# jspenmar/slowtv_monodepth

Hardware: AMD Instinct MI355X
Metric: training images/sec (640×192, 3-frame) at 1/2/4/8 MI355X; warp+SSIM HBM GB/s (higher is better)
Workload: dtype f32

## Files before the change

slowtv_monodepth_amd/csrc/smd_conv_stem.hip:

```cpp
#include "smd_common.h"
#include "smd_kernels.h"
#include "smd_conv_mfma_dev.h"
#include <algorithm>

namespace smd {

namespace {

template <int C> struct StemFwd {
  static constexpr int NI = 7*C, NS = (NI + 1)/2;
  static constexpr int PR = 13, PD = 67, PITCH = 68;
  static constexpr int PLANE = C*PR*PITCH, ITEMS = C*PR*PD;
};

template <int C>
__global__ __launch_bounds__(256) void k_stem_pack_w(const float* __restrict__ w, uint4* __restrict__ wp) {
  using T = StemFwd<C>;
  const int idx = blockIdx.x*256 + threadIdx.x;
  if (idx >= 2*T::NS*64) return;
  const int lane = idx & 63, s = (idx >> 6) % T::NS, mt = idx/(64*T::NS);
  const int i = 2*s + (lane >> 5), co = mt*32 + (lane & 31);
  float v[8];
#pragma unroll
  for (int kx = 0; kx < 8; ++kx) v[kx] = (i < T::NI && kx < 7) ? w[((size_t)co*T::NI + i)*7 + kx] : 0.f;
  unsigned pk[4][3];
#pragma unroll
  for (int q = 0; q < 4; ++q) split_pair<3>(v[2*q], v[2*q + 1], pk[q]);
#pragma unroll
  for (int p = 0; p < 3; ++p) wp[((size_t)(mt*T::NS + s)*3 + p)*64 + lane] = uint4{pk[0][p], pk[1][p], pk[2][p], pk[3][p]};
}

template <int C>
__global__ __launch_bounds__(256, 2) void k_stem_fwd(const float* __restrict__ x, const uint4* __restrict__ wp, float* __restrict__ y, int H, int W, int ho, int wo) {
  using T = StemFwd<C>;
  constexpr int NS = T::NS, NI = T::NI, PR = T::PR, PD = T::PD, PITCH = T::PITCH, PLANE = T::PLANE, ITEMS = T::ITEMS;
  __shared__ __attribute__((aligned(16))) unsigned xs[3*PLANE];
  const int lane = threadIdx.x & 63, wv = __builtin_amdgcn_readfirstlane(threadIdx.x >> 6), j = lane & 31, g = lane >> 5;
  const int x0 = blockIdx.x*64, y0 = blockIdx.y*4, b = blockIdx.z;
  const float* xb = x + (size_t)b*C*H*W;

  for (int base = 0; base < ITEMS; base += 1024) {
    float v[4][2];
#pragma unroll
    for (int u = 0; u < 4; ++u) {
      const int item = base + u*256 + (int)threadIdx.x;
      const int d = item % PD, r = (item/PD) % PR, c = item/(PD*PR);
      const int gy = 2*y0 - 3 + r, gx = 2*x0 - 3 + 2*d;
      const bool ok = item < ITEMS && gy >= 0 && gy < H;
      v[u][0] = (ok && gx >= 0 && gx < W) ? xb[((size_t)c*H + gy)*W + gx] : 0.f;
      v[u][1] = (ok && gx + 1 >= 0 && gx + 1 < W) ? xb[((size_t)c*H + gy)*W + gx + 1] : 0.f;
    }
#pragma unroll
    for (int u = 0; u < 4; ++u) {
      const int item = base + u*256 + (int)threadIdx.x;
      if (item < ITEMS) {
        const int d = item % PD, rc = item/PD;
        unsigned pk[3];
        split_pair<3>(v[u][0], v[u][1], pk);
#pragma unroll
        for (int p = 0; p < 3; ++p) xs[p*PLANE + rc*PITCH + d] = pk[p];
      }
    }
  }
  __syncthreads();

  f32x16 acc[2][2], lo[2][2];
#pragma unroll
  for (int mt = 0; mt < 2; ++mt)
#pragma unroll
    for (int nf = 0; nf < 2; ++nf)
#pragma unroll
      for (int r = 0; r < 16; ++r) { acc[mt][nf][r] = 0.f; lo[mt][nf][r] = 0.f; }

  const uint4* wl = wp + lane;
  uint4 an[2][3];
#pragma unroll
  for (int mt = 0; mt < 2; ++mt)
#pragma unroll
    for (int p = 0; p < 3; ++p) an[mt][p] = wl[((mt*NS + 0)*3 + p)*64];
#pragma unroll
  for (int s = 0; s < NS; ++s) {
    bf16x8 A[2][3];
#pragma unroll
    for (int mt = 0; mt < 2; ++mt)
#pragma unroll
      for (int p = 0; p < 3; ++p) A[mt][p] = as_frag(an[mt][p]);
    const int sn = min(s + 1, NS - 1);
#pragma unroll
    for (int mt = 0; mt < 2; ++mt)
#pragma unroll
      for (int p = 0; p < 3; ++p) an[mt][p] = wl[((mt*NS + sn)*3 + p)*64];
    const int i = min(2*s + g, NI - 1);
    const int c = i/7, ky = i - 7*c;
    const unsigned* row = xs + (c*PR + 2*wv + ky)*PITCH + j;
    bf16x8 Bf[2][3];
#pragma unroll
    for (int nf = 0; nf < 2; ++nf)
#pragma unroll
      for (int p = 0; p < 3; ++p) {
        const unsigned* q = row + p*PLANE + nf*32;
        Bf[nf][p] = as_frag(uint4{q[0], q[1], q[2], q[3]});
      }
    split_mfma<3>(A, Bf, acc, lo);
  }

  const int yy = y0 + wv;
  if (yy >= ho) return;
#pragma unroll
  for (int mt = 0; mt < 2; ++mt)
#pragma unroll
    for (int nf = 0; nf < 2; ++nf) {
      const int xx = x0 + nf*32 + j;
      if (xx < wo) {
#pragma unroll
        for (int r = 0; r < 16; ++r) {
          const int co = mt*32 + mfma32_row(r, g);
          y[(((size_t)b*64 + co)*ho + yy)*wo + xx] = acc[mt][nf][r] + lo[mt][nf][r];
        }
      }
    }
}

template <int C> struct StemWgrad {
  static constexpr int NW = 49*C, NT = (NW + 31)/32, NTW = (NT + 1)/2;
  static constexpr int XP = 34, GP = 36;
  static constexpr int XPLANE = C*8*2*XP, GPLANE = 64*GP;
  static constexpr int XITEMS = C*2*XP, XTR = (XITEMS + 255)/256;
};

template <int C>
__global__ __launch_bounds__(256, 2) void k_stem_wgrad(const float* __restrict__ x, const float* __restrict__ gy, float* __restrict__ partial,
                                                       int H, int W, int ho, int wo, int rows_per_block) {
  using T = StemWgrad<C>;
  constexpr int NW = T::NW, NT = T::NT, NTW = T::NTW, XP = T::XP, GP = T::GP, XPLANE = T::XPLANE, GPLANE = T::GPLANE, XITEMS = T::XITEMS, XTR = T::XTR;
  constexpr int NPROD = n_products(3);
  __shared__ __attribute__((aligned(16))) unsigned xs[3*XPLANE];
  __shared__ __attribute__((aligned(16))) unsigned gs[3*GPLANE];
  const int lane = threadIdx.x & 63, wv = __builtin_amdgcn_readfirstlane(threadIdx.x >> 6), j = lane & 31, g = lane >> 5;
  const int mt = wv & 1, nh = wv >> 1;
  const int x0 = blockIdx.x*64, ybeg = blockIdx.y*rows_per_block, nrows = min(rows_per_block, ho - ybeg), b = blockIdx.z;
  const float* xb = x + (size_t)b*C*H*W;
  const float* gb = gy + (size_t)b*64*ho*wo;

  int xoff[NTW], sh[NTW], kyv[NTW];
#pragma unroll
  for (int i = 0; i < NTW; ++i) {
    const int n = min((nh + 2*i)*32 + j, NW - 1);
    const int c = n/49, rem = n - 49*c, ky = rem/7, kx = rem - 7*ky;
    xoff[i] = (c*16 + ((kx & 1) ^ 1))*XP; sh[i] = (kx + 1) >> 1; kyv[i] = ky;
  }

  float xv[XTR][4], gv[4][4];
  auto load_x = [&](int ir0) {
#pragma unroll
    for (int t = 0; t < XTR; ++t) {
      const int item = t*256 + (int)threadIdx.x;
      const int d = item % XP, rr = (item/XP) & 1, c = item/(2*XP);
      const int ir = ir0 + rr, gc = 2*x0 - 4 + 4*d;
      const bool ok = item < XITEMS && ir >= 0 && ir < H;
#pragma unroll
      for (int k = 0; k < 4; ++k) xv[t][k] = (ok && gc + k >= 0 && gc + k < W) ? xb[((size_t)c*H + ir)*W + gc + k] : 0.f;
    }
  };
  auto file_x = [&](int ir0) {
#pragma unroll
    for (int t = 0; t < XTR; ++t) {
      const int item = t*256 + (int)threadIdx.x;
      if (item < XITEMS) {
        const int d = item % XP, rr = (item/XP) & 1, c = item/(2*XP);
        const int slot = (ir0 + rr + 8) & 7;
        unsigned pe[3], po[3];
        split_pair<3>(xv[t][0], xv[t][2], pe);
        split_pair<3>(xv[t][1], xv[t][3], po);
#pragma unroll
        for (int p = 0; p < 3; ++p) {
          xs[p*XPLANE + ((c*8 + slot)*2 + 0)*XP + d] = pe[p];
          xs[p*XPLANE + ((c*8 + slot)*2 + 1)*XP + d] = po[p];
        }
      }
    }
  };
  auto load_g = [&](int yy) {
#pragma unroll
    for (int t = 0; t < 4; ++t) {
      const int item = t*256 + (int)threadIdx.x;
      const int co = item >> 4, xa = x0 + 4*(item & 15);
#pragma unroll
      for (int k = 0; k < 4; ++k) gv[t][k] = (xa + k < wo) ? gb[((size_t)co*ho + yy)*wo + xa + k] : 0.f;
    }
  };
  auto file_g = [&]() {
#pragma unroll
    for (int t = 0; t < 4; ++t) {
      const int item = t*256 + (int)threadIdx.x;
      const int co = item >> 4, q = item & 15;
      unsigned p0[3], p1[3];
      split_pair<3>(gv[t][0], gv[t][1], p0);
      split_pair<3>(gv[t][2], gv[t][3], p1);
#pragma unroll
      for (int p = 0; p < 3; ++p) {
        gs[p*GPLANE + co*GP + 2*q] = p0[p];
        gs[p*GPLANE + co*GP + 2*q + 1] = p1[p];
      }
    }
  };

  f32x16 acc[NTW];
#pragma unroll
  for (int i = 0; i < NTW; ++i)
#pragma unroll
    for (int r = 0; r < 16; ++r) acc[i][r] = 0.f;

  for (int k = 0; k < 4; ++k) { load_x(2*ybeg - 4 + 2*k); file_x(2*ybeg - 4 + 2*k); }
  load_g(ybeg); file_g();
  __syncthreads();
  for (int r = 0; r < nrows; ++r) {
    const int yy = ybeg + r;
    const bool more = r + 1 < nrows;
    if (more) { load_x(2*yy + 4); load_g(yy + 1); }
    unsigned rowa[NTW];
#pragma unroll
    for (int i = 0; i < NTW; ++i) rowa[i] = (unsigned)(xoff[i] + ((2*yy + 5 + kyv[i]) & 7)*2*XP);
#pragma unroll
    for (int ks = 0; ks < 4; ++ks) {
      bf16x8 A[3];
#pragma unroll
      for (int p = 0; p < 3; ++p) A[p] = as_frag(*reinterpret_cast<const uint4*>(&gs[p*GPLANE + (mt*32 + j)*GP + ks*8 + g*4]));
#pragma unroll
      for (int i = 0; i < NTW; ++i) {
        if (nh + 2*i >= NT) continue;
        const int e = ks*16 + g*8 + sh[i];
        const unsigned* q = xs + rowa[i] + (e >> 1);
        const unsigned s16 = (unsigned)(e & 1)*16u;
        bf16x8 Bf[3];
#pragma unroll
        for (int p = 0; p < 3; ++p) {
          const unsigned d0 = q[p*XPLANE], d1 = q[p*XPLANE + 1], d2 = q[p*XPLANE + 2], d3 = q[p*XPLANE + 3], d4 = q[p*XPLANE + 4];
          Bf[p] = as_frag(uint4{__builtin_amdgcn_alignbit(d1, d0, s16), __builtin_amdgcn_alignbit(d2, d1, s16),
                                __builtin_amdgcn_alignbit(d3, d2, s16), __builtin_amdgcn_alignbit(d4, d3, s16)});
        }
#pragma unroll
        for (int t = 0; t < NPROD; ++t) acc[i] = mfma_bf16(A[prod_a(3, t)], Bf[prod_b(3, t)], acc[i]);
      }
    }
    __syncthreads();
    if (more) { file_x(2*yy + 4); file_g(); }
    __syncthreads();
  }

  const size_t blk = ((size_t)b*gridDim.y + blockIdx.y)*gridDim.x + blockIdx.x;
#pragma unroll
  for (int i = 0; i < NTW; ++i) {
    const int nt = nh + 2*i, n = nt*32 + j;
    if (nt < NT && n < NW) {
#pragma unroll
      for (int r = 0; r < 16; ++r) {
        const int co = mt*32 + mfma32_row(r, g);
        partial[(blk*64 + co)*NW + n] = acc[i][r];
      }
    }
  }
}

void stem_wgrad_shape(int B, int ho, int wo, dim3& grid, int& rows) {
  const int strips = ceil_div(wo, 64);
  const long long units = (long long)strips*B;
  const int groups = (int)std::max(1ll, std::min<long long>(ceil_div(ho, 8), 512/std::max(units, 1ll)));
  rows = ceil_div(ho, groups);
  grid = dim3(strips, ceil_div(ho, rows), B);
}

}

bool conv_stem_served(int C, int CO) { return CO == 64 && (C == 3 || C == 6); }
size_t conv_stem_packed_bytes(int C) { return (size_t)2*((7*C + 1)/2)*3*1024; }
size_t conv_stem_wgrad_floats(int B, int C, int H, int W) {
  dim3 grid; int rows;
  stem_wgrad_shape(B, (H - 1)/2 + 1, (W - 1)/2 + 1, grid, rows);
  return partial_sets_floats(grid.x*grid.y*grid.z, (size_t)64*49*C);
}
hipError_t launch_conv_stem_pack(const float* w, void* wp, int C, hipStream_t st) {
  const int n = 2*((7*C + 1)/2)*64;
  if (C == 3) hipLaunchKernelGGL(k_stem_pack_w<3>, dim3(ceil_div(n, 256)), dim3(256), 0, st, w, (uint4*)wp);
  else hipLaunchKernelGGL(k_stem_pack_w<6>, dim3(ceil_div(n, 256)), dim3(256), 0, st, w, (uint4*)wp);
  return hipGetLastError();
}
hipError_t launch_conv_stem_fwd(const float* x, const void* wp, float* y, int B, int C, int H, int W, hipStream_t st) {
  const int ho = (H - 1)/2 + 1, wo = (W - 1)/2 + 1;
  const dim3 grid(ceil_div(wo, 64), ceil_div(ho, 4), B);
  if (C == 3) hipLaunchKernelGGL(k_stem_fwd<3>, grid, dim3(256), 0, st, x, (const uint4*)wp, y, H, W, ho, wo);
  else hipLaunchKernelGGL(k_stem_fwd<6>, grid, dim3(256), 0, st, x, (const uint4*)wp, y, H, W, ho, wo);
  return hipGetLastError();
}
hipError_t launch_conv_stem_bwd_wgt(const float* x, const float* gy, float* g_w, float* partial, int B, int C, int H, int W, hipStream_t st) {
  const int ho = (H - 1)/2 + 1, wo = (W - 1)/2 + 1, n = 64*49*C;
  dim3 grid; int rows;
  stem_wgrad_shape(B, ho, wo, grid, rows);
  if (C == 3) hipLaunchKernelGGL(k_stem_wgrad<3>, grid, dim3(256), 0, st, x, gy, partial, H, W, ho, wo, rows);
  else hipLaunchKernelGGL(k_stem_wgrad<6>, grid, dim3(256), 0, st, x, gy, partial, H, W, ho, wo, rows);
  return launch_partial_sets_finalize(partial, grid.x*grid.y*grid.z, n, SetIndexMap{}, g_w, st);
}

}
```

Baseline: 953.8.

## Restructure stem conv kernels: triple-buffered weight prefetch, split odd tile, compact row ring

In the stem forward kernel, the input tile staging loop is fully unrolled. Weight fragments are now prefetched two steps ahead through a three-slot register ring, with scheduling barriers around the MFMA step. In the weight-gradient kernel, the x row ring shrinks from 8 slots to 5 row pairs, and global loads are made unconditional through clamped addresses, with masking moved to the LDS fill. The A fragments for all k-steps are hoisted before the MFMA loop. When the tile count is odd, the last tile's k-steps are split across the two wave halves and combined through LDS. These changes aim to balance MFMA work across waves and overlap global loads with compute, at the cost of more registers and extra barriers.

Result: no change. 955.9, median of 3 (+0.2%).

```diff
diff --git a/slowtv_monodepth_amd/csrc/smd_conv_stem.hip b/slowtv_monodepth_amd/csrc/smd_conv_stem.hip
--- a/slowtv_monodepth_amd/csrc/smd_conv_stem.hip
+++ b/slowtv_monodepth_amd/csrc/smd_conv_stem.hip
@@ -10,7 +10,7 @@
 template <int C> struct StemFwd {
   static constexpr int NI = 7*C, NS = (NI + 1)/2;
   static constexpr int PR = 13, PD = 67, PITCH = 68;
-  static constexpr int PLANE = C*PR*PITCH, ITEMS = C*PR*PD;
+  static constexpr int PLANE = C*PR*PITCH, ITEMS = C*PR*PD, TRIPS = (ITEMS + 255)/256;
 };
 
 template <int C>
@@ -33,30 +33,30 @@
 template <int C>
 __global__ __launch_bounds__(256, 2) void k_stem_fwd(const float* __restrict__ x, const uint4* __restrict__ wp, float* __restrict__ y, int H, int W, int ho, int wo) {
   using T = StemFwd<C>;
-  constexpr int NS = T::NS, NI = T::NI, PR = T::PR, PD = T::PD, PITCH = T::PITCH, PLANE = T::PLANE, ITEMS = T::ITEMS;
+  constexpr int NS = T::NS, NI = T::NI, PR = T::PR, PD = T::PD, PITCH = T::PITCH, PLANE = T::PLANE, ITEMS = T::ITEMS, TRIPS = T::TRIPS;
   __shared__ __attribute__((aligned(16))) unsigned xs[3*PLANE];
   const int lane = threadIdx.x & 63, wv = __builtin_amdgcn_readfirstlane(threadIdx.x >> 6), j = lane & 31, g = lane >> 5;
   const int x0 = blockIdx.x*64, y0 = blockIdx.y*4, b = blockIdx.z;
   const float* xb = x + (size_t)b*C*H*W;
 
-  for (int base = 0; base < ITEMS; base += 1024) {
-    float v[4][2];
-#pragma unroll
-    for (int u = 0; u < 4; ++u) {
-      const int item = base + u*256 + (int)threadIdx.x;
+  {
+    float v[TRIPS][2];
+#pragma unroll
+    for (int t = 0; t < TRIPS; ++t) {
+      const int item = t*256 + (int)threadIdx.x;
       const int d = item % PD, r = (item/PD) % PR, c = item/(PD*PR);
       const int gy = 2*y0 - 3 + r, gx = 2*x0 - 3 + 2*d;
       const bool ok = item < ITEMS && gy >= 0 && gy < H;
-      v[u][0] = (ok && gx >= 0 && gx < W) ? xb[((size_t)c*H + gy)*W + gx] : 0.f;
-      v[u][1] = (ok && gx + 1 >= 0 && gx + 1 < W) ? xb[((size_t)c*H + gy)*W + gx + 1] : 0.f;
-    }
-#pragma unroll
-    for (int u = 0; u < 4; ++u) {
-      const int item = base + u*256 + (int)threadIdx.x;
+      v[t][0] = (ok && gx >= 0 && gx < W) ? xb[((size_t)c*H + gy)*W + gx] : 0.f;
+      v[t][1] = (ok && gx + 1 >= 0 && gx + 1 < W) ? xb[((size_t)c*H + gy)*W + gx + 1] : 0.f;
+    }
+#pragma unroll
+    for (int t = 0; t < TRIPS; ++t) {
+      const int item = t*256 + (int)threadIdx.x;
       if (item < ITEMS) {
         const int d = item % PD, rc = item/PD;
         unsigned pk[3];
-        split_pair<3>(v[u][0], v[u][1], pk);
+        split_pair<3>(v[t][0], v[t][1], pk);
 #pragma unroll
         for (int p = 0; p < 3; ++p) xs[p*PLANE + rc*PITCH + d] = pk[p];
       }
@@ -73,23 +73,17 @@
       for (int r = 0; r < 16; ++r) { acc[mt][nf][r] = 0.f; lo[mt][nf][r] = 0.f; }
 
   const uint4* wl = wp + lane;
-  uint4 an[2][3];
-#pragma unroll
-  for (int mt = 0; mt < 2; ++mt)
-#pragma unroll
-    for (int p = 0; p < 3; ++p) an[mt][p] = wl[((mt*NS + 0)*3 + p)*64];
+  bf16x8 A[3][2][3];
+  auto fetch_a = [&](bf16x8 (&dst)[2][3], int s) {
+#pragma unroll
+    for (int mt = 0; mt < 2; ++mt)
+#pragma unroll
+      for (int p = 0; p < 3; ++p) dst[mt][p] = as_frag(wl[((mt*NS + s)*3 + p)*64]);
+  };
+  fetch_a(A[0], 0); fetch_a(A[1], 1);
 #pragma unroll
   for (int s = 0; s < NS; ++s) {
-    bf16x8 A[2][3];
-#pragma unroll
-    for (int mt = 0; mt < 2; ++mt)
-#pragma unroll
-      for (int p = 0; p < 3; ++p) A[mt][p] = as_frag(an[mt][p]);
-    const int sn = min(s + 1, NS - 1);
-#pragma unroll
-    for (int mt = 0; mt < 2; ++mt)
-#pragma unroll
-      for (int p = 0; p < 3; ++p) an[mt][p] = wl[((mt*NS + sn)*3 + p)*64];
+    if (s + 2 < NS) fetch_a(A[(s + 2) % 3], s + 2);
     const int i = min(2*s + g, NI - 1);
     const int c = i/7, ky = i - 7*c;
     const unsigned* row = xs + (c*PR + 2*wv + ky)*PITCH + j;
@@ -101,7 +95,8 @@
         const unsigned* q = row + p*PLANE + nf*32;
         Bf[nf][p] = as_frag(uint4{q[0], q[1], q[2], q[3]});
       }
-    split_mfma<3>(A, Bf, acc, lo);
+    split_mfma<3>(A[s % 3], Bf, acc, lo);
+    __builtin_amdgcn_sched_barrier(0);
   }
 
   const int yy = y0 + wv;
@@ -123,8 +118,10 @@
 
 template <int C> struct StemWgrad {
   static constexpr int NW = 49*C, NT = (NW + 31)/32, NTW = (NT + 1)/2;
+  static constexpr bool SPLIT = NT & 1;
   static constexpr int XP = 34, GP = 36;
-  static constexpr int XPLANE = C*8*2*XP, GPLANE = 64*GP;
+  static constexpr int RP = 5;
+  static constexpr int XPLANE = C*RP*2*2*XP, GPLANE = 64*GP;
   static constexpr int XITEMS = C*2*XP, XTR = (XITEMS + 255)/256;
 };
 
@@ -132,7 +129,8 @@
 __global__ __launch_bounds__(256, 2) void k_stem_wgrad(const float* __restrict__ x, const float* __restrict__ gy, float* __restrict__ partial,
                                                        int H, int W, int ho, int wo, int rows_per_block) {
   using T = StemWgrad<C>;
-  constexpr int NW = T::NW, NT = T::NT, NTW = T::NTW, XP = T::XP, GP = T::GP, XPLANE = T::XPLANE, GPLANE = T::GPLANE, XITEMS = T::XITEMS, XTR = T::XTR;
+  constexpr int NW = T::NW, NT = T::NT, NTW = T::NTW, XP = T::XP, GP = T::GP, XPLANE = T::XPLANE, GPLANE = T::GPLANE, XITEMS = T::XITEMS, XTR = T::XTR, RP = T::RP;
+  constexpr bool SPLIT = T::SPLIT;
   constexpr int NPROD = n_products(3);
   __shared__ __attribute__((aligned(16))) unsigned xs[3*XPLANE];
   __shared__ __attribute__((aligned(16))) unsigned gs[3*GPLANE];
@@ -142,12 +140,13 @@
   const float* xb = x + (size_t)b*C*H*W;
   const float* gb = gy + (size_t)b*64*ho*wo;
 
-  int xoff[NTW], sh[NTW], kyv[NTW];
+  auto tile_of = [&](int i) { return (SPLIT && i == NTW - 1) ? NT - 1 : nh + 2*i; };
+  int xoff[NTW], sh[NTW], dpair[NTW];
 #pragma unroll
   for (int i = 0; i < NTW; ++i) {
-    const int n = min((nh + 2*i)*32 + j, NW - 1);
+    const int n = min(tile_of(i)*32 + j, NW - 1);
     const int c = n/49, rem = n - 49*c, ky = rem/7, kx = rem - 7*ky;
-    xoff[i] = (c*16 + ((kx & 1) ^ 1))*XP; sh[i] = (kx + 1) >> 1; kyv[i] = ky;
+    xoff[i] = ((c*RP*2 + ((ky + 1) & 1))*2 + ((kx & 1) ^ 1))*XP; sh[i] = (kx + 1) >> 1; dpair[i] = RP + ((ky - 3) >> 1);
   }
 
   float xv[XTR][4], gv[4][4];
@@ -157,25 +156,29 @@
       const int item = t*256 + (int)threadIdx.x;
       const int d = item % XP, rr = (item/XP) & 1, c = item/(2*XP);
       const int ir = ir0 + rr, gc = 2*x0 - 4 + 4*d;
-      const bool ok = item < XITEMS && ir >= 0 && ir < H;
-#pragma unroll
-      for (int k = 0; k < 4; ++k) xv[t][k] = (ok && gc + k >= 0 && gc + k < W) ? xb[((size_t)c*H + ir)*W + gc + k] : 0.f;
-    }
-  };
-  auto file_x = [&](int ir0) {
+      const float* row = xb + ((size_t)min(c, C - 1)*H + min(max(ir, 0), H - 1))*W;
+#pragma unroll
+      for (int k = 0; k < 4; ++k) xv[t][k] = row[min(max(gc + k, 0), W - 1)];
+    }
+  };
+  auto file_x = [&](int ir0, int slot) {
 #pragma unroll
     for (int t = 0; t < XTR; ++t) {
       const int item = t*256 + (int)threadIdx.x;
       if (item < XITEMS) {
         const int d = item % XP, rr = (item/XP) & 1, c = item/(2*XP);
-        const int slot = (ir0 + rr + 8) & 7;
+        const int ir = ir0 + rr, gc = 2*x0 - 4 + 4*d;
+        const bool ok = ir >= 0 && ir < H;
+        float z[4];
+#pragma unroll
+        for (int k = 0; k < 4; ++k) z[k] = (ok && gc + k >= 0 && gc + k < W) ? xv[t][k] : 0.f;
         unsigned pe[3], po[3];
-        split_pair<3>(xv[t][0], xv[t][2], pe);
-        split_pair<3>(xv[t][1], xv[t][3], po);
+        split_pair<3>(z[0], z[2], pe);
+        split_pair<3>(z[1], z[3], po);
 #pragma unroll
         for (int p = 0; p < 3; ++p) {
-          xs[p*XPLANE + ((c*8 + slot)*2 + 0)*XP + d] = pe[p];
-          xs[p*XPLANE + ((c*8 + slot)*2 + 1)*XP + d] = po[p];
+          xs[p*XPLANE + (((c*RP + slot)*2 + rr)*2 + 0)*XP + d] = pe[p];
+          xs[p*XPLANE + (((c*RP + slot)*2 + rr)*2 + 1)*XP + d] = po[p];
         }
       }
     }
@@ -186,17 +189,20 @@
       const int item = t*256 + (int)threadIdx.x;
       const int co = item >> 4, xa = x0 + 4*(item & 15);
 #pragma unroll
-      for (int k = 0; k < 4; ++k) gv[t][k] = (xa + k < wo) ? gb[((size_t)co*ho + yy)*wo + xa + k] : 0.f;
+      for (int k = 0; k < 4; ++k) gv[t][k] = gb[((size_t)co*ho + yy)*wo + min(xa + k, wo - 1)];
     }
   };
   auto file_g = [&]() {
 #pragma unroll
     for (int t = 0; t < 4; ++t) {
       const int item = t*256 + (int)threadIdx.x;
-      const int co = item >> 4, q = item & 15;
+      const int co = item >> 4, q = item & 15, xa = x0 + 4*q;
+      float z[4];
+#pragma unroll
+      for (int k = 0; k < 4; ++k) z[k] = (xa + k < wo) ? gv[t][k] : 0.f;
       unsigned p0[3], p1[3];
-      split_pair<3>(gv[t][0], gv[t][1], p0);
-      split_pair<3>(gv[t][2], gv[t][3], p1);
+      split_pair<3>(z[0], z[1], p0);
+      split_pair<3>(z[2], z[3], p1);
 #pragma unroll
       for (int p = 0; p < 3; ++p) {
         gs[p*GPLANE + co*GP + 2*q] = p0[p];
@@ -211,24 +217,33 @@
 #pragma unroll
     for (int r = 0; r < 16; ++r) acc[i][r] = 0.f;
 
-  for (int k = 0; k < 4; ++k) { load_x(2*ybeg - 4 + 2*k); file_x(2*ybeg - 4 + 2*k); }
+  int ym = ybeg % RP;
+  for (int k = 0; k < 4; ++k) { load_x(2*ybeg - 4 + 2*k); file_x(2*ybeg - 4 + 2*k, (ym + RP - 2 + k) % RP); }
   load_g(ybeg); file_g();
   __syncthreads();
   for (int r = 0; r < nrows; ++r) {
     const int yy = ybeg + r;
     const bool more = r + 1 < nrows;
+    bf16x8 A[4][3];
+#pragma unroll
+    for (int ks = 0; ks < 4; ++ks)
+#pragma unroll
+      for (int p = 0; p < 3; ++p) A[ks][p] = as_frag(*reinterpret_cast<const uint4*>(&gs[p*GPLANE + (mt*32 + j)*GP + ks*8 + g*4]));
     if (more) { load_x(2*yy + 4); load_g(yy + 1); }
+    __syncthreads();
+    __builtin_amdgcn_sched_barrier(0);
     unsigned rowa[NTW];
 #pragma unroll
-    for (int i = 0; i < NTW; ++i) rowa[i] = (unsigned)(xoff[i] + ((2*yy + 5 + kyv[i]) & 7)*2*XP);
+    for (int i = 0; i < NTW; ++i) {
+      int slot = ym + dpair[i];
+      slot -= slot >= RP ? RP : 0; slot -= slot >= RP ? RP : 0;
+      rowa[i] = (unsigned)(xoff[i] + slot*4*XP);
+    }
 #pragma unroll
     for (int ks = 0; ks < 4; ++ks) {
-      bf16x8 A[3];
-#pragma unroll
-      for (int p = 0; p < 3; ++p) A[p] = as_frag(*reinterpret_cast<const uint4*>(&gs[p*GPLANE + (mt*32 + j)*GP + ks*8 + g*4]));
 #pragma unroll
       for (int i = 0; i < NTW; ++i) {
-        if (nh + 2*i >= NT) continue;
+        if (SPLIT && i == NTW - 1 && (ks >> 1) != nh) continue;
         const int e = ks*16 + g*8 + sh[i];
         const unsigned* q = xs + rowa[i] + (e >> 1);
         const unsigned s16 = (unsigned)(e & 1)*16u;
@@ -240,19 +255,33 @@
                                 __builtin_amdgcn_alignbit(d3, d2, s16), __builtin_amdgcn_alignbit(d4, d3, s16)});
         }
 #pragma unroll
-        for (int t = 0; t < NPROD; ++t) acc[i] = mfma_bf16(A[prod_a(3, t)], Bf[prod_b(3, t)], acc[i]);
-      }
-    }
+        for (int t = 0; t < NPROD; ++t) acc[i] = mfma_bf16(A[ks][prod_a(3, t)], Bf[prod_b(3, t)], acc[i]);
+      }
+    }
+    __builtin_amdgcn_sched_barrier(0);
+    if (more) { file_x(2*yy + 4, (ym + 2) % RP); file_g(); }
     __syncthreads();
-    if (more) { file_x(2*yy + 4); file_g(); }
+    ym = ym + 1 == RP ? 0 : ym + 1;
+  }
+
+  if constexpr (SPLIT) {
+    float* red = reinterpret_cast<float*>(gs);
+    if (nh == 1) {
+#pragma unroll
+      for (int r = 0; r < 16; ++r) red[(mt*16 + r)*64 + lane] = acc[NTW - 1][r];
+    }
     __syncthreads();
+    if (nh == 0) {
+#pragma unroll
+      for (int r = 0; r < 16; ++r) acc[NTW - 1][r] += red[(mt*16 + r)*64 + lane];
+    }
   }
 
   const size_t blk = ((size_t)b*gridDim.y + blockIdx.y)*gridDim.x + blockIdx.x;
 #pragma unroll
   for (int i = 0; i < NTW; ++i) {
-    const int nt = nh + 2*i, n = nt*32 + j;
-    if (nt < NT && n < NW) {
+    const int nt = tile_of(i), n = nt*32 + j;
+    if (nt < NT && n < NW && !(SPLIT && i == NTW - 1 && nh == 1)) {
 #pragma unroll
       for (int r = 0; r < 16; ++r) {
         const int co = mt*32 + mfma32_row(r, g);
```
